# team-ergo-unipi/ergo_uvo

Hardware: AMD Instinct MI355X
Metric: stereo frame-pairs/sec (detect+match+pose) @1920x1080, 3k kpts (higher is better)
Workload: dtype f32+f64

## Files before the change

ergo_uvo_amd/csrc/ctx.hip:

```cpp
#include "uvo_ctx.h"
#include "uvo_pix.h"
#include <pthread.h>
#include "uvo_epnp.h"
#include <string.h>
#include <sched.h>
#include <atomic>
#include <math.h>
#include <float.h>
#include <new>
#include <algorithm>
namespace uvo { extern bool g_bdbg; extern std::atomic<double> g_bstat[16]; double now_us(); void operator+=(std::atomic<double>& a, double v); }

using namespace uvo;

struct uvo_ctx : public uvo::Ctx {};

namespace {
uvo_status abi_caught(uvo_ctx* c) noexcept
{
    uvo_status st = UVO_HIP_ERROR;
    const char* what = "unexpected C++ exception inside libuvo_hip";
    static thread_local char text[160];
    try { throw; }
    catch (const std::bad_alloc&) { st = UVO_CAPACITY; what = "out of host memory (std::bad_alloc) inside libuvo_hip"; }
// ... 116 lines not shown
static int stereo_a_streams(const uvo::Ctx* m, int depth) { return a_per_lane(m, depth) ? depth : a_shared_streams(m); }
static int stereo_a_slot(const uvo::Ctx* m, int depth, int lane, long long launch) { return a_per_lane(m, depth) ? lane : (int)(launch % a_shared_streams(m)); }
static void assign_entry_streams(uvo::Ctx* m, uvo::Ctx* L, bool stereo)
{
    if (L->assigned_seq == m->sh->plan_seq) return;
    L->assigned_seq = m->sh->plan_seq;
    const int depth = (int)m->sh->lanes.size();
    if (!stereo) { L->stream = slot_stream(m, 0, L->lane_id); L->pnp_stream = slot_stream(m, 1, L->lane_id); return; }
    L->stream = slot_stream(m, 0, stereo_a_slot(m, depth, L->lane_id, m->sh->a_launch++));
    L->pnp_stream = slot_stream(m, 1, m->sh->shared_slots ? (int)(m->sh->plan_seq % m->sh->n_b) : L->lane_id);
}
static void assign_idle_streams(uvo::Ctx* m)
{
    const int depth = (int)m->sh->lanes.size();
    m->sh->shared_slots = shared_layout(depth);
    m->sh->n_b = std::min((int)Shared::kMaxDepth, m->sh->max_b + 1);
    if (const char* e = getenv("UVO_B_STREAMS")) m->sh->n_b = std::min((int)Shared::kMaxDepth, std::max(1, atoi(e)));
    m->sh->a_launch = 0;
    if (m->sh->shared_slots) for (int i = 0; i < m->sh->n_b; i++) (void)slot_stream(m, 1, i);
    for (uvo::Ctx* l : m->sh->lanes) {
        l->stream = slot_stream(m, 0, stereo_a_slot(m, depth, l->lane_id, l->lane_id));
        l->pnp_stream = slot_stream(m, 1, m->sh->shared_slots ? l->lane_id % m->sh->n_b : l->lane_id);
        l->assigned_seq = -1;
    }
}

static const char* unsupported_params(const uvo_params* p)
{
    if (p->ITERATIONS_COUNT > 0 && p->PNP_METHOD_FLAG != 1)
        return "PNP_METHOD_FLAG: uvo_params takes only 1 (cv::SOLVEPNP_EPNP, the value shipped in stereo_VO_parameters.yaml); 2 (P3P), 3 (DLS) and 4 (UPNP) "
               "are set with uvo_ctx_set_pnp_method, 0 (ITERATIVE), 5 (AP3P) and above are not implemented";
    if (p->USE_EXTRINSIC_GUESS != 0) return "USE_EXTRINSIC_GUESS: only false is implemented (EPnP ignores the guess)";
    return nullptr;
}

static thread_local const char* t_create_refusal = nullptr;

static uvo_status create_one(const uvo_params* p, int device, int max_w, int max_h, int max_kpts, uvo_ctx** out, int lane = 0, Shared* sh = nullptr)
{
    if (!out) return UVO_INVALID_ARG;
    *out = nullptr;
    t_create_refusal = p ? unsupported_params(p) : nullptr;
    if (!p || max_w < 16 || max_h < 16 || max_kpts < 16 || t_create_refusal) return UVO_INVALID_ARG;
    int ndev = 0;
    if (hipGetDeviceCount(&ndev) != hipSuccess || ndev <= 0 || device < 0 || device >= ndev) return UVO_NO_DEVICE;
    if (hipSetDevice(device) != hipSuccess) return UVO_HIP_ERROR;
    uvo_ctx* c = new (std::nothrow) uvo_ctx();
    if (!c) return UVO_HIP_ERROR;
    c->sh = sh ? sh : new (std::nothrow) Shared();
    if (!c->sh) { delete c; return UVO_HIP_ERROR; }
    c->p = *p; c->device = device; c->max_w = max_w; c->max_h = max_h; c->cap = max_kpts; c->lane_id = lane;
    const size_t cap = (size_t)max_kpts;
    const size_t npx = (size_t)max_w * max_h, nsum = (size_t)(max_w + 1) * (max_h + 1);
    const int nstrip = (max_h + 7) / 8;
    c->colpart_stride = ((max_w + 1 + 2047) / 2048) * 2048;
    const size_t nchunks = (cap + 127) / 128;
    hipError_t e = hipSuccess;
#define A(expr) do { if (e == hipSuccess) e = (expr); } while (0)
    if (lane != 0) { c->stream = c->sh->slot_streams[0][0]; c->pnp_stream = c->sh->slot_streams[1][0]; }
    else { A(stream_acquire(device, 0, 0, &c->sh->slot_streams[0][0])); c->stream = c->sh->slot_streams[0][0]; }
    A(hipEventCreate(&c->ev0)); A(hipEventCreate(&c->ev1));
    c->plane_pw = ((max_w + 1 + 3) / 4 + 1 + 1) & ~1;
    c->plane_stride = c->plane_pw * ((max_h + 1 + 3) / 4 + 1);
    for (int i = 0; i < 2; i++) {
        A(dalloc(&c->d_planes[i], (size_t)16 * c->plane_stride));
        if (e == hipSuccess) e = hipMemset(c->d_planes[i], 0, sizeof(int32_t) * 16 * c->plane_stride);
        A(dalloc(&c->d_img[i], npx)); A(dalloc(&c->d_sum_base[i], nsum + 2 * kSumPad));
        if (e == hipSuccess) { e = hipMemset(c->d_sum_base[i], 0, sizeof(int32_t) * (nsum + 2 * kSumPad)); c->d_sum[i] = c->d_sum_base[i] + kSumPad; }
        A(dalloc(&c->d_cand[i], cap)); A(dalloc(&c->det[i].kps, cap)); A(dalloc(&c->det[i].desc, cap * 128));
        A(dalloc(&c->d_tmp_desc[i], cap * 128)); A(dalloc(&c->d_matches[i], cap));
        A(dalloc(&c->d_as_kpsL[i], cap)); A(dalloc(&c->d_as_kpsR[i], cap)); A(dalloc(&c->d_as_descL[i], cap * 128));
        A(dalloc(&c->d_as_pts4[i], cap)); A(dalloc(&c->d_as_cam1[i], cap * 3)); A(dalloc(&c->d_as_flag[i], cap));
    }
    c->surv_cap = 4 * (int)cap; A(dalloc(&c->d_surv, (size_t)c->surv_cap));
    A(dalloc(&c->d_colpart, (size_t)2 * nstrip * c->colpart_stride));
    A(dalloc(&c->d_DW, 400)); A(dalloc(&c->d_rank, cap * 2)); A(dalloc(&c->d_big_par, cap * 4)); A(dalloc(&c->d_big_patch, cap * 2 * 448));
    A(dalloc(&c->d_mpart, 2 * nchunks * cap)); A(dalloc(&c->d_mscratch, 2 * (nchunks + 4))); A(dalloc(&c->d_knn_idx, 2 * cap * 2)); A(dalloc(&c->d_knn_dist, 2 * cap * 2));
    A(dalloc(&c->d_x1, cap)); A(dalloc(&c->d_x2, cap)); A(dalloc(&c->d_xc, cap)); A(dalloc(&c->d_pts4, cap));
    A(dalloc(&c->d_cam1, cap * 3)); A(dalloc(&c->d_flag, cap)); A(dalloc(&c->d_tmp_idx, cap)); A(dalloc(&c->d_tmp_row, cap));
    if (const char* ww = getenv("UVO_WORKER_WAIT")) c->worker_wait = !strcmp(ww, "spin") ? 0 : (!strcmp(ww, "block-all") ? 2 : ((!strcmp(ww, "sleep") || !strcmp(ww, "block")) ? 3 : 1));
    c->wait_eff.store(c->worker_wait == 0 ? 0 : (c->worker_wait == 2 ? 2 : 1), std::memory_order_relaxed);
    A(hipEventCreateWithFlags(&c->evBlock, hipEventDisableTiming | hipEventBlockingSync));
    A(hipEventCreateWithFlags(&c->evPoll, hipEventDisableTiming));
    A(hipEventCreateWithFlags(&c->evB, hipEventDisableTiming | (c->worker_wait == 2 ? hipEventBlockingSync : 0)));
    for (int i = 0; i < 2; i++) {
        A(dalloc(&c->d_good_pts[i], cap * 3)); A(dalloc(&c->d_good_idx[i], cap));
        A(dalloc(&c->d_opts[i], cap * 3)); A(dalloc(&c->d_ipts[i], cap));
        A(hipEventCreateWithFlags(&c->evA[i], hipEventDisableTiming | ((i == 0 && c->worker_wait == 2) ? hipEventBlockingSync : 0)));
        A(hipHostMalloc(reinterpret_cast<void**>(&c->h_countsA[i]), sizeof(int) * CN_TOTAL));
    }
    A(hipEventCreateWithFlags(&c->evAS, hipEventDisableTiming));
    A(hipEventCreateWithFlags(&c->evSync, hipEventDisableTiming));
    A(hipEventCreateWithFlags(&c->evProducer, hipEventDisableTiming));
    A(hipEventCreateWithFlags(&c->evDet, hipEventDisableTiming)); A(hipEventCreateWithFlags(&c->evPrevRead, hipEventDisableTiming));
    if (lane == 0) { A(stream_acquire(device, 1, 0, &c->sh->slot_streams[1][0])); c->pnp_stream = c->sh->slot_streams[1][0]; }
    A(dalloc(&c->d_countsB, (size_t)4)); A(hipHostMalloc(reinterpret_cast<void**>(&c->h_countsB), sizeof(int) * 4));
    A(dalloc(&c->d_counts, (size_t)CN_TOTAL));
    A(dalloc(&c->d_subsets, (size_t)kMaxHyp * 5)); A(dalloc(&c->d_models, (size_t)kMaxHyp * 6)); A(dalloc(&c->d_hcount, (size_t)kMaxHyp));
    A(dalloc(&c->d_inliers, cap)); A(dalloc(&c->d_refit, cap * 21)); A(dalloc(&c->d_pose, (size_t)6));
    A(hipHostMalloc(reinterpret_cast<void**>(&c->h_counts), sizeof(int) * CN_TOTAL));
    A(hipHostMalloc(reinterpret_cast<void**>(&c->h_subsets), sizeof(int) * kMaxHyp * 5));
    A(hipHostMalloc(reinterpret_cast<void**>(&c->h_hcount), sizeof(int) * kMaxHyp));
    A(hipHostMalloc(reinterpret_cast<void**>(&c->h_pose), sizeof(double) * 6));
    A(dalloc(&c->d_rng_raw, (size_t)1024)); A(hipMalloc(&c->d_spec, 64)); A(hipHostMalloc(&c->h_spec, 64));
#undef A
    if (e != hipSuccess) { destroy_one(c); return UVO_HIP_ERROR; }
    c->d_cand_n = c->d_counts + CN_CAND0;
    c->det[0].n = c->d_counts + CN_NL; c->det[1].n = c->d_counts + CN_NR;
    c->d_nmatch = c->d_counts + CN_M;
    c->d_as_n = c->d_counts + CN_AS0;
    c->d_big_n = c->d_counts + CN_BIG0;
    if (surf_build_area_tables(c) != UVO_OK) { destroy_one(c); return UVO_HIP_ERROR; }
    {
        std::vector<unsigned> raw(1024);
        uint64_t state = (uint64_t)-1;
        for (auto& v : raw) v = rng_next(state);
        if (hipMemcpy(c->d_rng_raw, raw.data(), sizeof(unsigned) * raw.size(), hipMemcpyHostToDevice) != hipSuccess ||
            hipMemset(c->d_spec, 0, 64) != hipSuccess) { destroy_one(c); return UVO_HIP_ERROR; }
        memset(c->h_spec, 0, 64);
    }
    make_desc_weights(c->h_DW);
    if (hipMemcpy(c->d_DW, c->h_DW, sizeof(float) * 400, hipMemcpyHostToDevice) != hipSuccess ||
        hipMemset(c->d_rank, 0, sizeof(int) * cap * 2) != hipSuccess ||
        hipMemset(c->d_counts, 0, sizeof(int) * CN_TOTAL) != hipSuccess) { destroy_one(c); return UVO_HIP_ERROR; }
    if (getenv("UVO_TRACE") && trace_alloc(c) != hipSuccess) { destroy_one(c); return UVO_HIP_ERROR; }
    try { c->err.reserve(256); c->worker = std::thread(lane_worker, c); }
    catch (...) { destroy_one(c); return UVO_HIP_ERROR; }
    *out = c;
// ... 123 lines not shown
    if (st != UVO_OK) { uvo_ctx* made = *out; *out = nullptr; destroy_ctx(made); }
    return st;
} UVO_ABI_CATCH(nullptr)

extern "C" uvo_status uvo_stereo_set_depth(uvo_ctx* c, int depth)
try {
    if (!c) return UVO_INVALID_ARG;
    (void)hipSetDevice(c->device);
    return set_depth(c, depth);
} UVO_ABI_CATCH(c)

static void destroy_ctx(uvo_ctx* c)
{
    if (uvo::g_bdbg && uvo::g_bstat[4].load() > 0) {
        const double n = uvo::g_bstat[4].load();
        fprintf(stderr, "[uvo] stage B over %.0f calls, host wall us per call: wait-for-A %.1f | hyp+score to sync %.1f | host scan + refit launch %.1f | refit to sync %.1f | semaphore wait %.1f\n",
                n, uvo::g_bstat[0].load() / n, uvo::g_bstat[1].load() / n, uvo::g_bstat[2].load() / n, uvo::g_bstat[3].load() / n, uvo::g_bstat[5].load() / n);
        fprintf(stderr, "[uvo] uvo_stereo_submit host wall: %.1f us per pair over %.0f pairs\n", uvo::g_bstat[6].load() / std::max(1.0, uvo::g_bstat[7].load()), uvo::g_bstat[7].load());
        const double np = std::max(1.0, uvo::g_bstat[7].load());
        fprintf(stderr, "[uvo]   of which: upload %.1f | a_overlap wait %.1f | detector launches %.1f | matcher .. extract_3Dpoints launches %.1f\n",
                uvo::g_bstat[8].load() / np, uvo::g_bstat[9].load() / np, uvo::g_bstat[10].load() / np, uvo::g_bstat[11].load() / np);
    }
    write_trace(c);
    for (size_t i = c->sh->lanes.size(); i > 1; i--) destroy_one(static_cast<uvo_ctx*>(c->sh->lanes[i - 1]));
    c->sh->lanes.clear();
    destroy_one(c);
}
extern "C" void uvo_ctx_destroy(uvo_ctx* c)
try { if (c) destroy_ctx(c); } UVO_ABI_CATCH_VOID(c)

static void destroy_one(uvo_ctx* c)
{
    if (!c) return;
    (void)hipSetDevice(c->device);
    if (c->worker.joinable()) {
        { std::lock_guard<std::mutex> lk(c->mu); c->quit = true; }
        c->cv.notify_all();
        c->worker.join();
    }
    sync_owned_streams(c);
    for (int i = 0; i < 2; i++) {
        (void)hipFree(c->d_img[i]); (void)hipFree(c->d_sum_base[i]); (void)hipFree(c->d_planes[i]); (void)hipFree(c->d_cand[i]); (void)hipFree(c->det[i].kps);
        (void)hipFree(c->det[i].desc); (void)hipFree(c->d_tmp_desc[i]); (void)hipFree(c->d_matches[i]);
        (void)hipFree(c->d_as_kpsL[i]); (void)hipFree(c->d_as_kpsR[i]); (void)hipFree(c->d_as_descL[i]);
        (void)hipFree(c->d_as_pts4[i]); (void)hipFree(c->d_as_cam1[i]); (void)hipFree(c->d_as_flag[i]);
    }
    mono_ws_free(c);
    pre_ws_free(c);
    frames_ws_free(c);
    codec_ws_free(c);
    sift_ws_free(c);
    akaze_ws_free(c);
    orb_ws_free(c);
    void* ptrs[] = { c->d_hess_order, c->d_gen_tab, c->d_gen_planes, c->d_surv, c->d_octpat, c->d_colpart, c->d_DW, c->d_rank, c->d_big_par, c->d_big_patch, c->d_area_tabs, c->d_area_iscale, c->d_ori_w, c->d_mpart, c->d_mscratch, c->d_knn_idx, c->d_knn_dist, c->d_x1, c->d_x2, c->d_xc, c->d_pts4, c->d_cam1,
                     c->d_flag, c->d_tmp_idx, c->d_tmp_row, c->d_good_pts[0], c->d_good_pts[1], c->d_good_idx[0], c->d_good_idx[1], c->d_opts[0], c->d_opts[1],
                     c->d_ipts[0], c->d_ipts[1], c->d_counts, c->d_countsB, c->d_subsets, c->d_models,
                     c->d_hcount, c->d_inliers, c->d_refit, c->d_pose };
    for (void* p : ptrs) (void)hipFree(p);
    (void)hipHostFree(c->h_counts); (void)hipHostFree(c->h_subsets); (void)hipHostFree(c->h_hcount); (void)hipHostFree(c->h_pose);
    (void)hipHostFree(c->h_countsB); (void)hipHostFree(c->h_spec); (void)hipFree(c->d_rng_raw); (void)hipFree(c->d_spec);
    for (int i = 0; i < 2; i++) { (void)hipHostFree(c->h_countsA[i]); if (c->evA[i]) (void)hipEventDestroy(c->evA[i]); }
    if (c->evAS) (void)hipEventDestroy(c->evAS);
    if (c->evBlock) (void)hipEventDestroy(c->evBlock);
    if (c->evPoll) (void)hipEventDestroy(c->evPoll);
    if (c->evB) (void)hipEventDestroy(c->evB);
    if (c->evSync) (void)hipEventDestroy(c->evSync);
    if (c->evProducer) (void)hipEventDestroy(c->evProducer);
    for (auto& r : c->trace) for (int k = 0; k < 8; k++) if (r.ev[k]) (void)hipEventDestroy(r.ev[k]);
    if (c->evDet) (void)hipEventDestroy(c->evDet);
    if (c->evPrevRead) (void)hipEventDestroy(c->evPrevRead);
    if (c->ev0) (void)hipEventDestroy(c->ev0);
    if (c->ev1) (void)hipEventDestroy(c->ev1);
    if (c->lane_id == 0) {
        for (int role = 0; role < 2; role++) for (int i = 0; i < Shared::kMaxDepth; i++) { stream_release(c->device, role, i, c->sh->slot_streams[role][i]); c->sh->slot_streams[role][i] = nullptr; }
        delete c->sh;
    }
    delete c;
}

extern "C" const char* uvo_last_error(const uvo_ctx* c) { return c ? c->err.c_str() : (t_create_refusal ? t_create_refusal : "null context"); }
extern "C" void* uvo_ctx_stream(uvo_ctx* c) { return c ? (void*)c->stream : nullptr; }
extern "C" uvo_status uvo_ctx_set_params(uvo_ctx* c, const uvo_params* p)
try {
    if (!c || !p) return UVO_INVALID_ARG;
    if (c->sh->n_pending != 0) { c->err = "parameters cannot change while pairs are in flight"; return UVO_INVALID_ARG; }
    if (const char* why = unsupported_params(p)) { c->err = why; return UVO_INVALID_ARG; }
    if ((p->SURF_EXTENDED != 0) != (c->p.SURF_EXTENDED != 0) && (c->sh->vo_initialized || c->sh->mono_initialized)) {
        c->err = "SURF_EXTENDED changes the descriptor width: the previous frame's descriptors held by the running VO loop would not match (uvo_stereo_reset / uvo_mono_reset first)";
        return UVO_INVALID_ARG;
    }
    for (Ctx* l : c->sh->lanes) l->p = *p;
    return UVO_OK;
} UVO_ABI_CATCH(c)
extern "C" uvo_status uvo_ctx_set_producer_stream(uvo_ctx* c, void* hip_stream, int enabled)
try {
    if (!c) return UVO_INVALID_ARG;
    c->sh->producer_stream = static_cast<hipStream_t>(hip_stream); c->sh->has_producer = enabled != 0;
    return UVO_OK;
} UVO_ABI_CATCH(c)
extern "C" uvo_status uvo_device_alloc(uvo_ctx* c, size_t bytes, void** out)
try {
    if (!c) return UVO_INVALID_ARG;
    if (!out || bytes == 0) { c->err = "uvo_device_alloc: NULL result pointer or zero bytes"; return UVO_INVALID_ARG; }
    *out = nullptr;
    (void)hipSetDevice(c->device);
    UVO_HIP_TRY(c, hipMalloc(out, bytes));
    return UVO_OK;
// ... 2047 lines not shown
```

ergo_uvo_amd/csrc/surf.hip:

```cpp
#include "uvo_ctx.h"
#include <type_traits>
#include <string.h>
#include "uvo_math.h"
#include <algorithm>
#include <utility>
#include <vector>
#include <string>

namespace uvo {

struct ImgPair { const uint8_t* img[2]; int32_t* sum[2]; int32_t* planes[2]; int pw, pstride; int* cand_n; int* big_n; int* surv_n; };
struct AreaTab;
struct CandOut { uvo_keypoint* cand[2]; int* count; int cap; };
struct SurvOut { Survivor* list; int* count; int cap; };
static_assert(sizeof(Survivor) == 128, "a survivor record is 32 words");
struct SortArgs { const uvo_keypoint* cand[2]; const int* cand_n; uvo_keypoint* out[2]; int* out_n[2]; int* rank; int cap;
                  int4* big_par; int* big_n; int* gate_nqa; int gate_min_features; };
struct DescArgs { const uint8_t* img[2]; uvo_keypoint* kps[2]; float* desc[2]; const int* n[2]; const float* DW;
                  const int4* big_par; const int* big_n; const int* big_large; int cap;
                  const AreaTab* tabs; const int* iscale;
                  int extended;
                  const int32_t* sum[2]; const float* ori_w; int* ori_drop; };
struct LaneArgs { ImgPair ip; int32_t* part; SurvOut sv; CandOut out; SortArgs sa; DescArgs da; uint8_t* patch; const int4* big_in; int4* big_out; int* big_large; };
static const int kStripRows = 8;
static const int kStripCols = 2048;

__device__ __forceinline__ void strip_row_prefix(const uint8_t* img, int w, int h, int y0, int c0, int (*wt)[4], int (&carry)[kStripRows],
                                                 unsigned (&lo)[kStripRows], unsigned (&hi)[kStripRows], int (&E)[kStripRows])
{
    const int tid = threadIdx.x, lane = tid & 63, wv = tid >> 6;
    const bool vec8 = (w & 7) == 0;
#pragma unroll
    for (int r = 0; r < kStripRows; r++) {
        const int y = y0 + r;
        lo[r] = hi[r] = 0;
        if (y < h && c0 < w) {
            const uint8_t* src = img + (size_t)y * w + c0;
            if (vec8) { const uint2 v = *reinterpret_cast<const uint2*>(src); lo[r] = v.x; hi[r] = v.y; }
            else {
                for (int k = 0; k < 8; k++) if (c0 + k < w) { if (k < 4) lo[r] |= (unsigned)src[k] << (8 * k); else hi[r] |= (unsigned)src[k] << (8 * (k - 4)); }
            }
        }
    }
    int local[kStripRows], inc[kStripRows];
#pragma unroll
    for (int r = 0; r < kStripRows; r++) inc[r] = local[r] = (int)__builtin_amdgcn_sad_u8(lo[r], 0u, __builtin_amdgcn_sad_u8(hi[r], 0u, 0u));
#pragma unroll
    for (int r = 0; r < kStripRows; r++) {
        int v = inc[r];
        v += __builtin_amdgcn_update_dpp(0, v, 0x111, 0xf, 0xf, false);
        v += __builtin_amdgcn_update_dpp(0, v, 0x112, 0xf, 0xf, false);
        v += __builtin_amdgcn_update_dpp(0, v, 0x114, 0xf, 0xf, false);
        v += __builtin_amdgcn_update_dpp(0, v, 0x118, 0xf, 0xf, false);
        v += __builtin_amdgcn_update_dpp(0, v, 0x142, 0xa, 0xf, false);
        v += __builtin_amdgcn_update_dpp(0, v, 0x143, 0xc, 0xf, false);
        inc[r] = v;
    }
    if (lane == 63) {
#pragma unroll
        for (int r = 0; r < kStripRows; r++) wt[r][wv] = inc[r];
    }
    __syncthreads();
#pragma unroll
    for (int r = 0; r < kStripRows; r++) {
        const int t0 = wt[r][0], t1 = wt[r][1], t2 = wt[r][2], t3 = wt[r][3];
        const int base = carry[r] + (wv > 0 ? t0 : 0) + (wv > 1 ? t1 : 0) + (wv > 2 ? t2 : 0);
        E[r] = base + inc[r] - local[r];
        carry[r] += t0 + t1 + t2 + t3;
    }
}
__device__ __forceinline__ int packed_px(unsigned lo, unsigned hi, int k) { return (int)(((k < 4 ? lo : hi) >> (8 * (k & 3))) & 255u); }

__global__ __launch_bounds__(256) void k_integral_strip_sums(LaneArgs LA, int w, int h, int cstride, int nstrip)
{
    const ImgPair& ip = LA.ip; int32_t* part = LA.part;
    const int strip = blockIdx.x, im = blockIdx.y, tid = threadIdx.x;
    __shared__ int wt[kStripRows][4];
    int carry[kStripRows];
#pragma unroll
    for (int r = 0; r < kStripRows; r++) carry[r] = 0;
    int32_t* dst = part + ((size_t)im * nstrip + strip) * cstride;
    for (int cb = 0; cb <= w; cb += kStripCols) {
        unsigned lo[kStripRows], hi[kStripRows]; int E[kStripRows];
        strip_row_prefix(ip.img[im], w, h, strip * kStripRows, cb + 8 * tid, wt, carry, lo, hi, E);
        int cs[8] = {0, 0, 0, 0, 0, 0, 0, 0};
#pragma unroll
        for (int r = 0; r < kStripRows; r++) {
            int run = E[r];
#pragma unroll
            for (int k = 0; k < 8; k++) { cs[k] += run; run += packed_px(lo[r], hi[r], k); }
        }
        int4* d4 = reinterpret_cast<int4*>(dst + cb + 8 * tid);
        d4[0] = make_int4(cs[0], cs[1], cs[2], cs[3]); d4[1] = make_int4(cs[4], cs[5], cs[6], cs[7]);
        __syncthreads();
    }
    if (strip == 0 && tid == 0) { ip.cand_n[im] = 0; ip.big_n[im] = 0; if (im == 0) { *ip.surv_n = 0; ip.surv_n[CN_ORI_DROP - CN_SURV] = 0; } }
}

__global__ __launch_bounds__(256) void k_integral_strip_scan(LaneArgs LA, int cstride, int nstrip, int w)
{
    int32_t* part = LA.part;
    const int tid = threadIdx.x, xl = tid & 31, g = tid >> 5, x = blockIdx.x * 32 + xl, im = blockIdx.y;
    __shared__ int gsum[8][32];
    const int per = (nstrip + 7) / 8, s0 = g * per, s1 = min(nstrip, s0 + per);
    int32_t* p = part + (size_t)im * nstrip * cstride + x;
    const bool live = x <= w;
    int tot = 0;
#pragma unroll 8
    for (int sI = s0; sI < s1; sI++) tot += live ? p[(size_t)sI * cstride] : 0;
    gsum[g][xl] = tot;
    __syncthreads();
    int acc = 0;
    for (int k = 0; k < g; k++) acc += gsum[k][xl];
    if (!live) return;
#pragma unroll 8
    for (int sI = s0; sI < s1; sI++) { const int v = p[(size_t)sI * cstride]; p[(size_t)sI * cstride] = acc; acc += v; }
}

__global__ __launch_bounds__(256) void k_integral_strip_final(LaneArgs LA, int w, int h, int cstride, int nstrip)
{
    const ImgPair& ip = LA.ip; const int32_t* part = LA.part;
    const int strip = blockIdx.x, im = blockIdx.y, tid = threadIdx.x;
    const int sw = w + 1, y0 = strip * kStripRows;
    __shared__ int wt[kStripRows][4];
    __shared__ __align__(16) int rowbuf[kStripRows / 2][kStripCols];
    int carry[kStripRows];
#pragma unroll
    for (int r = 0; r < kStripRows; r++) carry[r] = 0;
    const int32_t* src = part + ((size_t)im * nstrip + strip) * cstride;
    int32_t* sum = ip.sum[im];
    int32_t* planes = ip.planes[im];
    for (int cb = 0; cb <= w; cb += kStripCols) {
        const int c0 = cb + 8 * tid;
        const int4* s4 = reinterpret_cast<const int4*>(src + c0);
        const int4 a0 = s4[0], a1 = s4[1];
        unsigned lo[kStripRows], hi[kStripRows]; int E[kStripRows];
        strip_row_prefix(ip.img[im], w, h, y0, c0, wt, carry, lo, hi, E);
        int acc[8] = { a0.x, a0.y, a0.z, a0.w, a1.x, a1.y, a1.z, a1.w };
#pragma unroll
        for (int half = 0; half < 2; half++) {
#pragma unroll
            for (int rr = 0; rr < kStripRows / 2; rr++) {
                const int r = half * (kStripRows / 2) + rr, ys = y0 + r + 1;
                int run = E[r];
#pragma unroll
                for (int k = 0; k < 8; k++) { acc[k] += run; run += packed_px(lo[r], hi[r], k); }
                int4* rb = reinterpret_cast<int4*>(&rowbuf[rr][8 * tid]);
                rb[0] = make_int4(acc[0], acc[1], acc[2], acc[3]); rb[1] = make_int4(acc[4], acc[5], acc[6], acc[7]);
                if (((r + 1) & 3) != 2 && ys <= h && c0 <= w) {
                    int32_t* pl = planes + (size_t)((ys & 3) * 4) * ip.pstride + (size_t)(ys >> 2) * ip.pw + (c0 >> 2);
                    if (c0 + 7 <= w) {
#pragma unroll
                        for (int rx = 0; rx < 4; rx++) if (rx != 2) *reinterpret_cast<int2*>(pl + (size_t)rx * ip.pstride) = make_int2(acc[rx], acc[rx + 4]);
                    } else {
#pragma unroll
                        for (int k = 0; k < 8; k++) if ((k & 3) != 2 && c0 + k <= w) pl[(size_t)(k & 3) * ip.pstride + (k >> 2)] = acc[k];
                    }
                }
            }
            __syncthreads();
#pragma unroll
            for (int rr = 0; rr < kStripRows / 2; rr++) {
                const int ys = y0 + half * (kStripRows / 2) + rr + 1;
                if (ys <= h) {
                    int32_t* drow = sum + (size_t)ys * sw + cb;
#pragma unroll
                    for (int j = 0; j < 8; j++) { const int xs = tid + 256 * j; if (cb + xs <= w) drow[xs] = rowbuf[rr][xs]; }
                }
            }
            __syncthreads();
        }
    }
    if (strip == 0) for (int x = tid; x < sw; x += 256) sum[x] = 0;
}

struct LayerPat {
    int dx1[10], dy1[10], dx2[10], dy2[10];
    float w[10];
    int size, margin, samples_i, samples_j;
};
struct OctavePat {
    LayerPat L[5];
    int step, rows, cols;
    int lo, hi;
    int nms_margin[3];
    int octave;
};

struct OctDims { struct { int samples_i, samples_j; } L[5]; int rows, cols, nms_margin[3], octave; };
struct HessDims { OctDims o[4]; };
static void make_pattern(int size, LayerPat* lp)
{
    static const int dx_s[3][5]  = { {0, 2, 3, 7, 1}, {3, 2, 6, 7, -2}, {6, 2, 9, 7, 1} };
    static const int dy_s[3][5]  = { {2, 0, 7, 3, 1}, {2, 3, 7, 6, -2}, {2, 6, 7, 9, 1} };
    static const int dxy_s[4][5] = { {1, 1, 4, 4, 1}, {5, 1, 8, 4, -1}, {1, 5, 4, 8, -1}, {5, 5, 8, 8, 1} };
    float ratio = (float)size / 9;
    for (int k = 0; k < 10; k++) {
        const int* s = k < 3 ? dx_s[k] : k < 6 ? dy_s[k - 3] : dxy_s[k - 6];
        int dx1 = cv_round_f(ratio * s[0]), dy1 = cv_round_f(ratio * s[1]);
        int dx2 = cv_round_f(ratio * s[2]), dy2 = cv_round_f(ratio * s[3]);
        lp->dx1[k] = dx1; lp->dy1[k] = dy1; lp->dx2[k] = dx2; lp->dy2[k] = dy2;
        lp->w[k] = s[4] / ((float)(dx2 - dx1) * (dy2 - dy1));
    }
    lp->size = size;
}

static void make_octave(int octave, int nOctaveLayers, int w, int h, OctavePat* op)
{
    int step = 1 << octave;
    op->step = step; op->rows = h / step; op->cols = w / step; op->octave = octave;
    op->lo = 0; op->hi = 0;
    for (int l = 0; l < 5; l++) {
        int size = (9 + 6 * l) << octave;
        LayerPat* lp = &op->L[l];
        make_pattern(size, lp);
        lp->margin = (size / 2) / step;
        bool fits = l < nOctaveLayers + 2 && size <= h && size <= w;
        lp->samples_i = fits ? 1 + (h - size) / step : 0;
        lp->samples_j = fits ? 1 + (w - size) / step : 0;
        int lo = -lp->margin * step, hi = lo + size;
// ... 1734 lines not shown
    }
    UVO_HIP_TRY(c, hipMalloc(reinterpret_cast<void**>(&c->d_area_tabs), tabs.size() * sizeof(AreaTab)));
    UVO_HIP_TRY(c, hipMalloc(reinterpret_cast<void**>(&c->d_area_iscale), isc.size() * sizeof(int)));
    UVO_HIP_TRY(c, hipMemcpy(c->d_area_tabs, tabs.data(), tabs.size() * sizeof(AreaTab), hipMemcpyHostToDevice));
    UVO_HIP_TRY(c, hipMemcpy(c->d_area_iscale, isc.data(), isc.size() * sizeof(int), hipMemcpyHostToDevice));
    {
        const int N = 2 * kOriRadius + 1;
        double t[N], sum = 0; float G[N], W[N * N];
        const double sigma = 2.5f, scale2X = -0.5 / (sigma * sigma);
        for (int i = 0; i < N; i++) { const double x = i - (N - 1) * 0.5; t[i] = exp(scale2X * x * x); sum += t[i]; }
        sum = 1. / sum;
        for (int i = 0; i < N; i++) G[i] = (float)(t[i] * sum);
        for (int i = 0; i < N; i++) for (int j = 0; j < N; j++) W[i * N + j] = G[i] * G[j];
        UVO_HIP_TRY(c, hipMalloc(reinterpret_cast<void**>(&c->d_ori_w), sizeof(W)));
        UVO_HIP_TRY(c, hipMemcpy(c->d_ori_w, W, sizeof(W), hipMemcpyHostToDevice));
    }
    return UVO_OK;
}

uvo_status surf_upload(Ctx* c, int slot, const uint8_t* gray, int w, int h, int stride, int mem)
{
    if (!gray || w <= 0 || h <= 0 || w > c->max_w || h > c->max_h || stride < w || slot < 0 || slot > 1) {
        c->err = "surf_upload: bad image geometry (w/h exceed the context's max_w/max_h?)";
        return UVO_INVALID_ARG;
    }
    if (slot == 1 && (w != c->img_w || h != c->img_h)) { c->err = "left/right image sizes differ"; return UVO_INVALID_ARG; }
    c->img_w = w; c->img_h = h;
    if (mem == UVO_MEM_DEVICE && stride == w && (reinterpret_cast<uintptr_t>(gray) & 15u) == 0) { c->img[slot] = gray; return UVO_OK; }
    UVO_HIP_TRY(c, hipMemcpy2DAsync(c->d_img[slot], w, gray, stride, w, h,
                                    mem == UVO_MEM_DEVICE ? hipMemcpyDeviceToDevice : hipMemcpyHostToDevice, c->stream));
    c->img[slot] = c->d_img[slot];
    return UVO_OK;
}

static LaneArgs lane_args(Ctx* c, int nimg, int gate_min_features)
{
    LaneArgs a;
    a.ip = ImgPair{ { c->img[0], c->img[1] }, { c->d_sum[0], c->d_sum[1] }, { c->d_planes[0], c->d_planes[1] }, c->plane_pw, c->plane_stride, c->d_cand_n, c->d_big_n, c->d_counts + CN_SURV };
    a.part = c->d_colpart;
    a.sv = SurvOut{ c->d_surv, c->d_counts + CN_SURV, c->surv_cap };
    a.out = CandOut{ { c->d_cand[0], c->d_cand[1] }, c->d_cand_n, c->cap };
    a.sa = SortArgs{ { c->d_cand[0], c->d_cand[1] }, c->d_cand_n, { c->det[0].kps, c->det[1].kps }, { c->det[0].n, c->det[1].n }, c->d_rank, c->cap, c->d_big_par, c->d_big_n,
                     gate_min_features >= 0 && nimg == 2 ? c->d_counts + CN_NQA : nullptr, gate_min_features };
    a.da = DescArgs{ { c->img[0], c->img[1] }, { c->det[0].kps, c->det[1].kps }, { c->det[0].desc, c->det[1].desc }, { c->det[0].n, c->det[1].n }, c->d_DW,
                     c->d_big_par + (size_t)2 * c->cap, c->d_big_n, c->d_counts + CN_BIGL0, c->cap,
                     c->d_area_tabs, c->d_area_iscale, c->p.SURF_EXTENDED ? 1 : 0, { c->d_sum[0], c->d_sum[1] }, c->d_ori_w, c->d_counts + CN_ORI_DROP };
    a.patch = c->d_big_patch;
    a.big_in = c->d_big_par; a.big_out = c->d_big_par + (size_t)2 * c->cap; a.big_large = c->d_counts + CN_BIGL0;
    return a;
}

static uvo_status surf_integral_launch(Ctx* c, const LaneArgs& LA, int nimg)
{
    const int w = c->img_w, h = c->img_h, sw = w + 1;
    const int nstrip = (h + kStripRows - 1) / kStripRows, cstride = c->colpart_stride;
    StageTimer t(c, ST_INTEGRAL);
    hipLaunchKernelGGL(k_integral_strip_sums, dim3(nstrip, nimg), dim3(256), 0, c->stream, LA, w, h, cstride, nstrip);
    hipLaunchKernelGGL(k_integral_strip_scan, dim3((sw + 31) / 32, nimg), dim3(256), 0, c->stream, LA, cstride, nstrip, w);
    hipLaunchKernelGGL(k_integral_strip_final, dim3(nstrip, nimg), dim3(256), 0, c->stream, LA, w, h, cstride, nstrip);
    UVO_HIP_TRY(c, hipGetLastError());
    return UVO_OK;
}
uvo_status surf_integral(Ctx* c, int nimg) { return surf_integral_launch(c, lane_args(c, nimg, -1), nimg); }

template <class K>
static hipError_t raise_dynamic_lds(const Ctx* c, K kern, size_t bytes, bool (&done)[64])
{
    bool& set = done[c->device & 63];
    if (set) return hipSuccess;
    const hipError_t e = hipFuncSetAttribute(reinterpret_cast<const void*>(kern), hipFuncAttributeMaxDynamicSharedMemorySize, (int)bytes);
    set = e == hipSuccess;
    return e;
}

struct MergedGrid { int nbx0, nb0, nbx1, nb1, nb23, total; P23Grid g; };
static const int kMergedTW0 = 64, kMergedTH0 = 32, kMergedTW1 = 32;
static MergedGrid merged_grid(const OctavePat* ops)
{
    constexpr int TW0 = kMergedTW0, TH0 = kMergedTH0, TW1 = kMergedTW1, TH1 = kO1TileRows;
    MergedGrid m;
    m.nbx0 = (ops[0].cols + TW0 - 3) / (TW0 - 2); m.nb0 = m.nbx0 * ((ops[0].rows + TH0 - 3) / (TH0 - 2));
    m.nbx1 = (ops[1].cols + TW1 - 3) / (TW1 - 2); m.nb1 = m.nbx1 * ((ops[1].rows + TH1 - 3) / (TH1 - 2));
    m.g.nbx2 = (ops[2].cols + 32 - 3) / (32 - 2); m.g.nb2 = m.g.nbx2 * ((ops[2].rows + 16 - 3) / (16 - 2));
    m.g.nbx3 = (ops[3].cols + 16 - 3) / (16 - 2); m.g.nb3 = m.g.nbx3 * ((ops[3].rows + 16 - 3) / (16 - 2));
    m.nb23 = m.g.nb2 + m.g.nb3; m.total = m.nb0 + m.nb1 + m.nb23;
    return m;
}

static bool general_path(const Ctx* c)
{
    return c->sh->surf_detection_path == 1 || c->p.SURF_OCTAVES_LAYERS != 3 || c->p.SURF_OCTAVES_NUMBER > 4;
}
static int widest_window(const Ctx* c, int w, int h)
{
    int win = 0;
    for (int o = 0; o < c->p.SURF_OCTAVES_NUMBER; o++)
        for (int l = 1; l <= c->p.SURF_OCTAVES_LAYERS; l++) {
            const int size = (9 + 6 * (l + 1)) << o;
            if (size > w || size > h) break;
            const float sc = (float)size * 1.2f / 9.0f;
            win = std::max(win, (int)((20 + 1) * sc));
        }
    return win;
}
static uvo_status general_prepare(Ctx* c, int w, int h)
{
    const int no = c->p.SURF_OCTAVES_NUMBER, nl = c->p.SURF_OCTAVES_LAYERS + 2;
    std::vector<unsigned char> raw(sizeof(GenTab), 0);
    GenTab* tab = reinterpret_cast<GenTab*>(raw.data());
    long long off = 0, need = 0;
    for (int o = 0; o < no; o++) for (int l = 0; l < nl; l++) {
        GenLayer* g = &tab->L[o * nl + l];
// ... 211 lines not shown
```

ergo_uvo_amd/csrc/uvo_ctx.h:

```cpp
#pragma once
#include <hip/hip_runtime.h>
#include <string>
#include <thread>
#include <mutex>
#include <condition_variable>
#include <atomic>
#include <vector>
#include <deque>
#include <stdint.h>
#include "../../include/uvo_hip.h"

namespace uvo {

#define UVO_HIP_TRY(c, expr)                                                                  \
    do {                                                                                      \
        hipError_t _e = (expr);                                                               \
        if (_e != hipSuccess) {                                                               \
            (c)->err = std::string(#expr) + ": " + hipGetErrorString(_e);                     \
            return UVO_HIP_ERROR;                                                             \
        }                                                                                     \
    } while (0)

#define UVO_TRY(expr)                                                                         \
    do { uvo_status _s = (expr); if (_s != UVO_OK) return _s; } while (0)

enum Stage {
    ST_INTEGRAL = 0, ST_HESSIAN_O0, ST_HESSIAN_O1, ST_HESSIAN_O2, ST_HESSIAN_O3, ST_SORT, ST_DESCRIPTOR, ST_MATCH, ST_MATCH_MERGE, ST_GATHER,
    ST_TRIANGULATE, ST_EXTRACT3D, ST_PNP_HYP, ST_PNP_SCORE, ST_PNP_REFIT, ST_COUNT
};
static const char* const kStageNames[ST_COUNT] = {
    "integral", "hessian_nms_o0", "hessian_nms_o1", "hessian_nms_o2", "hessian_nms_o3", "kp_sort", "descriptor64", "match_top2", "match_merge", "gather",
    "triangulate", "extract3d", "pnp_epnp5", "pnp_score", "pnp_refit"
};

enum { CN_T = 0, CN_G = 1, CN_NINL = 2, CN_NQA = 3, CN_NQB = 4, CN_MEFF = 5, CN_NL = 6, CN_NR = 7,
       CN_CAND0 = 8, CN_CAND1 = 9, CN_M = 10, CN_TRAW = 11, CN_AS0 = 12, CN_AS1 = 13, CN_BIG0 = 14, CN_BIG1 = 15, CN_SURV = 16, CN_BIGL0 = 17, CN_BIGL1 = 18, CN_ORI_DROP = 19, CN_TOTAL = 20 };
struct GateArgs { int mode; int* cn; int min_features, cap; int* as_curr_n; const int* as_prev_n; };

static const int kSumPad = 256;
static const int kMaxHyp = 2048;
static const int kBinRowWords = 16;

struct Survivor { int im, octave, L, i, j; float n9[27]; };

struct DetectSet {
    uvo_keypoint* kps;
    float* desc;
    int* n;
};

struct Ctx;
struct Shared {
    static const int kMaxDepth = 16;
    static const int kInflightMonoInit = -1, kInflightStereoInit = -2;
    std::vector<Ctx*> lanes;
    int next_lane = 0;
    int prev_lane = 0, prev_buf = 0;
    bool prev_sync = true;
    int inflight[kMaxDepth]; int n_pending = 0;
    long long n_submitted = 0, n_collected = 0;
    int last_lane = 0;
    long long plan_seq = 0;
    long long a_launch = 0;
    bool in_sync_step = false;
    int kp_hint = 0;
    bool vo_initialized = false;
    std::vector<uvo_dmatch> init_matches;
    bool rig_set = false;
    double t_prev_curr[3] = {0, 0, 0}, rvec[3] = {0, 0, 0}, tvec[3] = {0, 0, 0};
    std::deque<uvo_stereo_result> stereo_init_results;
    bool mono_cam_set = false, mono_initialized = false, mono_pipelined = false;
    int mono_use_essential = 1;
    double mono_R[9] = {1,0,0,0,1,0,0,0,1}, mono_t[3] = {0,0,0}, mono_SF = 1.0;
    std::deque<uvo_mono_result> mono_init_results;
    hipStream_t producer_stream = nullptr; bool has_producer = false;
    std::string warning, policy_text;
    double K_left[9], K_right[9], R_right[9], t_right[3], P_eye_left[12], P_right[12];
    double mono_K[9];
    int stage_b_mode = -1;
    double cpu_budget = 0;
    int a_overlap = 2;
    int a_overlap_mono = 4;
    int max_b = 3;
    int max_b_mono = 10;
    int detector = 0;
    int pnp_method = 1;
    int mono_pose_stage = 0;
    int surf_detection_path = 0;
    bool shared_slots = false;
    int n_b = 1;
    hipStream_t slot_streams[2][kMaxDepth] = {};
    std::mutex b_mu; std::condition_variable b_cv;
    int b_running = 0;
    long long b_seq = 0;
};

struct Ctx {
    uvo_params p;
    int device = 0, max_w = 0, max_h = 0, cap = 0;
    hipStream_t stream = nullptr;
    std::string err;
    hipEvent_t evProducer = nullptr;

    uint8_t* d_img[2] = {nullptr, nullptr};
    const uint8_t* img[2] = {nullptr, nullptr};
    int32_t* d_sum[2] = {nullptr, nullptr};
    int32_t* d_sum_base[2] = {nullptr, nullptr};
    int32_t* d_colpart = nullptr;
    int colpart_stride = 0;
    int32_t* d_planes[2] = {nullptr, nullptr};
    int plane_pw = 0, plane_stride = 0;
    uvo_keypoint* d_cand[2] = {nullptr, nullptr};
    int* d_cand_n = nullptr;
    Survivor* d_surv = nullptr; int surv_cap = 0;
    void* d_octpat = nullptr;
    std::vector<unsigned char> h_octpat;
    uint32_t* d_hess_order = nullptr; size_t d_hess_order_cap = 0;
    std::vector<uint32_t> h_hess_order; int hess_order_key[3] = {0, 0, 0};
    void* d_gen_tab = nullptr; std::vector<unsigned char> h_gen_tab;
    float* d_gen_planes = nullptr; size_t gen_planes_cap = 0; long long gen_img_floats = 0;
    int4* d_big_par = nullptr; int* d_big_n = nullptr;
    struct AreaTab* d_area_tabs = nullptr;
    float* d_ori_w = nullptr;
    int* d_area_iscale = nullptr;
    uint8_t* d_big_patch = nullptr;
    int* d_rank = nullptr;
    DetectSet det[2];
    int img_w = 0, img_h = 0;
    float h_DW[400];
    float* d_DW = nullptr;

    float4* d_mpart = nullptr;
    float* d_mscratch = nullptr;
    int* d_knn_idx = nullptr;  float* d_knn_dist = nullptr;
    float* d_tmp_desc[2] = {nullptr, nullptr};
    uvo_dmatch* d_matches[2] = {nullptr, nullptr};
    int* d_nmatch = nullptr;

    uvo_keypoint* d_as_kpsL[2] = {nullptr, nullptr};
    uvo_keypoint* d_as_kpsR[2] = {nullptr, nullptr};
    float* d_as_descL[2] = {nullptr, nullptr};
    int* d_as_n = nullptr;
    float4* d_as_pts4[2] = {nullptr, nullptr};  double* d_as_cam1[2] = {nullptr, nullptr};  int* d_as_flag[2] = {nullptr, nullptr};

    uvo_point2f *d_x1 = nullptr, *d_x2 = nullptr, *d_xc = nullptr;
    float4* d_pts4 = nullptr;
    double* d_cam1 = nullptr;
    int* d_flag = nullptr;
    double* d_good_pts[2] = {nullptr, nullptr};  int* d_good_idx[2] = {nullptr, nullptr};
    float* d_opts[2] = {nullptr, nullptr};  uvo_point2f* d_ipts[2] = {nullptr, nullptr};
    int* d_tmp_idx = nullptr;
    int* d_tmp_row = nullptr;
    int* d_counts = nullptr;
    int* h_counts = nullptr;

    int* d_subsets = nullptr;
    int* h_subsets = nullptr;
    double* d_models = nullptr;
    int* d_hcount = nullptr;  int* h_hcount = nullptr;
    int* d_inliers = nullptr;
    double* d_refit = nullptr;
// ... 221 lines not shown
```

Measured before the change: 3984.

## Restructure SURF integral image into two-pass grouped column-sum scheme with 16-bit partials

Replaces the three-kernel integral image pipeline (strip sums, strip scan, final) with two kernels. The first computes per-strip column sums inside groups of 16 strips in LDS and stores 16-bit intra-group prefixes plus group totals. The final kernel then reconstructs the column carry by summing the preceding group totals. It also narrows the partial buffers to uint16, which halves that traffic, and vectorizes the integral row stores with alignment handling. The carry reconstruction is redundant: each strip re-reads all earlier group totals, so the work grows with image height, and there is added edge-handling complexity.

```diff
diff --git a/ergo_uvo_amd/csrc/ctx.hip b/ergo_uvo_amd/csrc/ctx.hip
--- a/ergo_uvo_amd/csrc/ctx.hip
+++ b/ergo_uvo_amd/csrc/ctx.hip
@@ -192,7 +192,7 @@
     c->p = *p; c->device = device; c->max_w = max_w; c->max_h = max_h; c->cap = max_kpts; c->lane_id = lane;
     const size_t cap = (size_t)max_kpts;
     const size_t npx = (size_t)max_w * max_h, nsum = (size_t)(max_w + 1) * (max_h + 1);
-    const int nstrip = (max_h + 7) / 8;
+    const int nstrip = (max_h + kStripRows - 1) / kStripRows, ngroup = (nstrip + kStripGroup - 1) / kStripGroup;
     c->colpart_stride = ((max_w + 1 + 2047) / 2048) * 2048;
     const size_t nchunks = (cap + 127) / 128;
     hipError_t e = hipSuccess;
@@ -214,6 +214,7 @@
     }
     c->surv_cap = 4 * (int)cap; A(dalloc(&c->d_surv, (size_t)c->surv_cap));
     A(dalloc(&c->d_colpart, (size_t)2 * nstrip * c->colpart_stride));
+    A(dalloc(&c->d_coltot, (size_t)2 * ngroup * c->colpart_stride));
     A(dalloc(&c->d_DW, 400)); A(dalloc(&c->d_rank, cap * 2)); A(dalloc(&c->d_big_par, cap * 4)); A(dalloc(&c->d_big_patch, cap * 2 * 448));
     A(dalloc(&c->d_mpart, 2 * nchunks * cap)); A(dalloc(&c->d_mscratch, 2 * (nchunks + 4))); A(dalloc(&c->d_knn_idx, 2 * cap * 2)); A(dalloc(&c->d_knn_dist, 2 * cap * 2));
     A(dalloc(&c->d_x1, cap)); A(dalloc(&c->d_x2, cap)); A(dalloc(&c->d_xc, cap)); A(dalloc(&c->d_pts4, cap));
@@ -443,7 +444,7 @@
     sift_ws_free(c);
     akaze_ws_free(c);
     orb_ws_free(c);
-    void* ptrs[] = { c->d_hess_order, c->d_gen_tab, c->d_gen_planes, c->d_surv, c->d_octpat, c->d_colpart, c->d_DW, c->d_rank, c->d_big_par, c->d_big_patch, c->d_area_tabs, c->d_area_iscale, c->d_ori_w, c->d_mpart, c->d_mscratch, c->d_knn_idx, c->d_knn_dist, c->d_x1, c->d_x2, c->d_xc, c->d_pts4, c->d_cam1,
+    void* ptrs[] = { c->d_hess_order, c->d_gen_tab, c->d_gen_planes, c->d_surv, c->d_octpat, c->d_colpart, c->d_coltot, c->d_DW, c->d_rank, c->d_big_par, c->d_big_patch, c->d_area_tabs, c->d_area_iscale, c->d_ori_w, c->d_mpart, c->d_mscratch, c->d_knn_idx, c->d_knn_dist, c->d_x1, c->d_x2, c->d_xc, c->d_pts4, c->d_cam1,
                      c->d_flag, c->d_tmp_idx, c->d_tmp_row, c->d_good_pts[0], c->d_good_pts[1], c->d_good_idx[0], c->d_good_idx[1], c->d_opts[0], c->d_opts[1],
                      c->d_ipts[0], c->d_ipts[1], c->d_counts, c->d_countsB, c->d_subsets, c->d_models,
                      c->d_hcount, c->d_inliers, c->d_refit, c->d_pose };
diff --git a/ergo_uvo_amd/csrc/surf.hip b/ergo_uvo_amd/csrc/surf.hip
--- a/ergo_uvo_amd/csrc/surf.hip
+++ b/ergo_uvo_amd/csrc/surf.hip
@@ -21,14 +21,25 @@
                   const AreaTab* tabs; const int* iscale;
                   int extended;
                   const int32_t* sum[2]; const float* ori_w; int* ori_drop; };
-struct LaneArgs { ImgPair ip; int32_t* part; SurvOut sv; CandOut out; SortArgs sa; DescArgs da; uint8_t* patch; const int4* big_in; int4* big_out; int* big_large; };
-static const int kStripRows = 8;
+struct LaneArgs { ImgPair ip; uint16_t* part; SurvOut sv; CandOut out; SortArgs sa; DescArgs da; uint8_t* patch; const int4* big_in; int4* big_out; int* big_large; };
 static const int kStripCols = 2048;
-
-__device__ __forceinline__ void strip_row_prefix(const uint8_t* img, int w, int h, int y0, int c0, int (*wt)[4], int (&carry)[kStripRows],
-                                                 unsigned (&lo)[kStripRows], unsigned (&hi)[kStripRows], int (&E)[kStripRows])
-{
-    const int tid = threadIdx.x, lane = tid & 63, wv = tid >> 6;
+static const int kStripBufRows = 2;
+static const int kGroupCols = 128;
+static_assert(kStripRows % 4 == 0 && kStripRows % kStripBufRows == 0, "plane rows go by (r + 1) & 3; whole LDS batches");
+static_assert(kStripGroup * (kGroupCols / 8) == 256 && kStripGroup * kStripRows * 255 < 65536, "a thread per strip and column octet; a group's column sums fit 16 bits");
+
+__device__ __forceinline__ int wave_inclusive_scan(int v)
+{
+    v += __builtin_amdgcn_update_dpp(0, v, 0x111, 0xf, 0xf, false);
+    v += __builtin_amdgcn_update_dpp(0, v, 0x112, 0xf, 0xf, false);
+    v += __builtin_amdgcn_update_dpp(0, v, 0x114, 0xf, 0xf, false);
+    v += __builtin_amdgcn_update_dpp(0, v, 0x118, 0xf, 0xf, false);
+    v += __builtin_amdgcn_update_dpp(0, v, 0x142, 0xa, 0xf, false);
+    v += __builtin_amdgcn_update_dpp(0, v, 0x143, 0xc, 0xf, false);
+    return v;
+}
+__device__ __forceinline__ void strip_load(const uint8_t* img, int w, int h, int y0, int c0, unsigned (&lo)[kStripRows], unsigned (&hi)[kStripRows])
+{
     const bool vec8 = (w & 7) == 0;
 #pragma unroll
     for (int r = 0; r < kStripRows; r++) {
@@ -42,20 +53,15 @@
             }
         }
     }
+}
+__device__ __forceinline__ void strip_row_prefix(int (*wt)[4], int (&carry)[kStripRows], const unsigned (&lo)[kStripRows], const unsigned (&hi)[kStripRows], int (&E)[kStripRows])
+{
+    const int tid = threadIdx.x, lane = tid & 63, wv = tid >> 6;
     int local[kStripRows], inc[kStripRows];
 #pragma unroll
-    for (int r = 0; r < kStripRows; r++) inc[r] = local[r] = (int)__builtin_amdgcn_sad_u8(lo[r], 0u, __builtin_amdgcn_sad_u8(hi[r], 0u, 0u));
-#pragma unroll
-    for (int r = 0; r < kStripRows; r++) {
-        int v = inc[r];
-        v += __builtin_amdgcn_update_dpp(0, v, 0x111, 0xf, 0xf, false);
-        v += __builtin_amdgcn_update_dpp(0, v, 0x112, 0xf, 0xf, false);
-        v += __builtin_amdgcn_update_dpp(0, v, 0x114, 0xf, 0xf, false);
-        v += __builtin_amdgcn_update_dpp(0, v, 0x118, 0xf, 0xf, false);
-        v += __builtin_amdgcn_update_dpp(0, v, 0x142, 0xa, 0xf, false);
-        v += __builtin_amdgcn_update_dpp(0, v, 0x143, 0xc, 0xf, false);
-        inc[r] = v;
-    }
+    for (int r = 0; r < kStripRows; r++) local[r] = (int)__builtin_amdgcn_sad_u8(lo[r], 0u, __builtin_amdgcn_sad_u8(hi[r], 0u, 0u));
+#pragma unroll
+    for (int r = 0; r < kStripRows; r++) inc[r] = wave_inclusive_scan(local[r]);
     if (lane == 63) {
 #pragma unroll
         for (int r = 0; r < kStripRows; r++) wt[r][wv] = inc[r];
@@ -71,77 +77,84 @@
 }
 __device__ __forceinline__ int packed_px(unsigned lo, unsigned hi, int k) { return (int)(((k < 4 ? lo : hi) >> (8 * (k & 3))) & 255u); }
 
-__global__ __launch_bounds__(256) void k_integral_strip_sums(LaneArgs LA, int w, int h, int cstride, int nstrip)
-{
-    const ImgPair& ip = LA.ip; int32_t* part = LA.part;
-    const int strip = blockIdx.x, im = blockIdx.y, tid = threadIdx.x;
+__global__ __launch_bounds__(256) void k_integral_group_sums(LaneArgs LA, uint16_t* tot16, int w, int h, int cstride, int nstrip, int ngroup)
+{
+    const ImgPair& ip = LA.ip; uint16_t* part16 = LA.part;
+    const int tid = threadIdx.x, t = tid & (kGroupCols / 8 - 1), sl = tid / (kGroupCols / 8);
+    const int group = blockIdx.x, im = blockIdx.z, strip = group * kStripGroup + sl, c0 = blockIdx.y * kGroupCols + 8 * t;
+    __shared__ uint4 colsum[kStripGroup][kGroupCols / 8];
+    unsigned lo[kStripRows], hi[kStripRows];
+    strip_load(ip.img[im], w, h, strip * kStripRows, c0, lo, hi);
+    uint4 own = make_uint4(0u, 0u, 0u, 0u);
+#pragma unroll
+    for (int r = 0; r < kStripRows; r++) {
+        own.x += lo[r] & 0x00ff00ffu; own.y += (lo[r] >> 8) & 0x00ff00ffu;
+        own.z += hi[r] & 0x00ff00ffu; own.w += (hi[r] >> 8) & 0x00ff00ffu;
+    }
+    colsum[sl][t] = own;
+    __syncthreads();
+    uint4 a = make_uint4(0u, 0u, 0u, 0u);
+#pragma unroll
+    for (int k = 0; k < kStripGroup - 1; k++) if (k < sl) { const uint4 v = colsum[k][t]; a.x += v.x; a.y += v.y; a.z += v.z; a.w += v.w; }
+    if (c0 < w) {
+        if (strip < nstrip) *reinterpret_cast<uint4*>(part16 + ((size_t)im * nstrip + strip) * cstride + c0) = a;
+        if (sl == kStripGroup - 1) *reinterpret_cast<uint4*>(tot16 + ((size_t)im * ngroup + group) * cstride + c0) = make_uint4(a.x + own.x, a.y + own.y, a.z + own.z, a.w + own.w);
+    }
+    if (group == 0 && blockIdx.y == 0 && tid == 0) { ip.cand_n[im] = 0; ip.big_n[im] = 0; if (im == 0) { *ip.surv_n = 0; ip.surv_n[CN_ORI_DROP - CN_SURV] = 0; } }
+}
+
+__global__ __launch_bounds__(256) void k_integral_strip_final(LaneArgs LA, const uint16_t* tot16, int w, int h, int cstride, int nstrip, int ngroup)
+{
+    const ImgPair& ip = LA.ip;
+    const int strip = blockIdx.x, im = blockIdx.y, tid = threadIdx.x, wv = tid >> 6;
+    const int sw = w + 1, y0 = strip * kStripRows, group = strip / kStripGroup;
     __shared__ int wt[kStripRows][4];
-    int carry[kStripRows];
+    __shared__ int wtv[4];
+    __shared__ __align__(16) int rowbuf[kStripBufRows][kStripCols];
+    int carry[kStripRows], carryv = 0;
 #pragma unroll
     for (int r = 0; r < kStripRows; r++) carry[r] = 0;
-    int32_t* dst = part + ((size_t)im * nstrip + strip) * cstride;
-    for (int cb = 0; cb <= w; cb += kStripCols) {
-        unsigned lo[kStripRows], hi[kStripRows]; int E[kStripRows];
-        strip_row_prefix(ip.img[im], w, h, strip * kStripRows, cb + 8 * tid, wt, carry, lo, hi, E);
-        int cs[8] = {0, 0, 0, 0, 0, 0, 0, 0};
-#pragma unroll
-        for (int r = 0; r < kStripRows; r++) {
-            int run = E[r];
-#pragma unroll
-            for (int k = 0; k < 8; k++) { cs[k] += run; run += packed_px(lo[r], hi[r], k); }
-        }
-        int4* d4 = reinterpret_cast<int4*>(dst + cb + 8 * tid);
-        d4[0] = make_int4(cs[0], cs[1], cs[2], cs[3]); d4[1] = make_int4(cs[4], cs[5], cs[6], cs[7]);
-        __syncthreads();
-    }
-    if (strip == 0 && tid == 0) { ip.cand_n[im] = 0; ip.big_n[im] = 0; if (im == 0) { *ip.surv_n = 0; ip.surv_n[CN_ORI_DROP - CN_SURV] = 0; } }
-}
-
-__global__ __launch_bounds__(256) void k_integral_strip_scan(LaneArgs LA, int cstride, int nstrip, int w)
-{
-    int32_t* part = LA.part;
-    const int tid = threadIdx.x, xl = tid & 31, g = tid >> 5, x = blockIdx.x * 32 + xl, im = blockIdx.y;
-    __shared__ int gsum[8][32];
-    const int per = (nstrip + 7) / 8, s0 = g * per, s1 = min(nstrip, s0 + per);
-    int32_t* p = part + (size_t)im * nstrip * cstride + x;
-    const bool live = x <= w;
-    int tot = 0;
-#pragma unroll 8
-    for (int sI = s0; sI < s1; sI++) tot += live ? p[(size_t)sI * cstride] : 0;
-    gsum[g][xl] = tot;
-    __syncthreads();
-    int acc = 0;
-    for (int k = 0; k < g; k++) acc += gsum[k][xl];
-    if (!live) return;
-#pragma unroll 8
-    for (int sI = s0; sI < s1; sI++) { const int v = p[(size_t)sI * cstride]; p[(size_t)sI * cstride] = acc; acc += v; }
-}
-
-__global__ __launch_bounds__(256) void k_integral_strip_final(LaneArgs LA, int w, int h, int cstride, int nstrip)
-{
-    const ImgPair& ip = LA.ip; const int32_t* part = LA.part;
-    const int strip = blockIdx.x, im = blockIdx.y, tid = threadIdx.x;
-    const int sw = w + 1, y0 = strip * kStripRows;
-    __shared__ int wt[kStripRows][4];
-    __shared__ __align__(16) int rowbuf[kStripRows / 2][kStripCols];
-    int carry[kStripRows];
-#pragma unroll
-    for (int r = 0; r < kStripRows; r++) carry[r] = 0;
-    const int32_t* src = part + ((size_t)im * nstrip + strip) * cstride;
+    const uint16_t* src16 = LA.part + ((size_t)im * nstrip + strip) * cstride;
+    const uint16_t* gtot16 = tot16 + (size_t)im * ngroup * cstride;
     int32_t* sum = ip.sum[im];
     int32_t* planes = ip.planes[im];
     for (int cb = 0; cb <= w; cb += kStripCols) {
         const int c0 = cb + 8 * tid;
-        const int4* s4 = reinterpret_cast<const int4*>(src + c0);
-        const int4 a0 = s4[0], a1 = s4[1];
         unsigned lo[kStripRows], hi[kStripRows]; int E[kStripRows];
-        strip_row_prefix(ip.img[im], w, h, y0, c0, wt, carry, lo, hi, E);
-        int acc[8] = { a0.x, a0.y, a0.z, a0.w, a1.x, a1.y, a1.z, a1.w };
-#pragma unroll
-        for (int half = 0; half < 2; half++) {
-#pragma unroll
-            for (int rr = 0; rr < kStripRows / 2; rr++) {
-                const int r = half * (kStripRows / 2) + rr, ys = y0 + r + 1;
+        strip_load(ip.img[im], w, h, y0, c0, lo, hi);
+        int V[8] = {0, 0, 0, 0, 0, 0, 0, 0};
+        if (c0 < w) {
+            for (int g0 = -1; g0 < group; g0 += 8) {
+                uint4 q[8];
+#pragma unroll
+                for (int k = 0; k < 8; k++) {
+                    const int g = g0 + k;
+                    q[k] = g < group ? *reinterpret_cast<const uint4*>(g < 0 ? src16 + c0 : gtot16 + (size_t)g * cstride + c0) : make_uint4(0u, 0u, 0u, 0u);
+                }
+#pragma unroll
+                for (int k = 0; k < 8; k++) {
+                    V[0] += (int)(q[k].x & 0xffffu); V[2] += (int)(q[k].x >> 16); V[1] += (int)(q[k].y & 0xffffu); V[3] += (int)(q[k].y >> 16);
+                    V[4] += (int)(q[k].z & 0xffffu); V[6] += (int)(q[k].z >> 16); V[5] += (int)(q[k].w & 0xffffu); V[7] += (int)(q[k].w >> 16);
+                }
+            }
+        }
+        const int vloc = V[0] + V[1] + V[2] + V[3] + V[4] + V[5] + V[6] + V[7], vinc = wave_inclusive_scan(vloc);
+        if ((tid & 63) == 63) wtv[wv] = vinc;
+        strip_row_prefix(wt, carry, lo, hi, E);
+        int acc[8];
+        {
+            const int t0 = wtv[0], t1 = wtv[1], t2 = wtv[2], t3 = wtv[3];
+            acc[0] = carryv + (wv > 0 ? t0 : 0) + (wv > 1 ? t1 : 0) + (wv > 2 ? t2 : 0) + vinc - vloc;
+#pragma unroll
+            for (int k = 1; k < 8; k++) acc[k] = acc[k - 1] + V[k - 1];
+            carryv += t0 + t1 + t2 + t3;
+        }
+        const int ncol = min(kStripCols, sw - cb);
+#pragma unroll
+        for (int part_i = 0; part_i < kStripRows / kStripBufRows; part_i++) {
+#pragma unroll
+            for (int rr = 0; rr < kStripBufRows; rr++) {
+                const int r = part_i * kStripBufRows + rr, ys = y0 + r + 1;
                 int run = E[r];
 #pragma unroll
                 for (int k = 0; k < 8; k++) { acc[k] += run; run += packed_px(lo[r], hi[r], k); }
@@ -160,12 +173,20 @@
             }
             __syncthreads();
 #pragma unroll
-            for (int rr = 0; rr < kStripRows / 2; rr++) {
-                const int ys = y0 + half * (kStripRows / 2) + rr + 1;
+            for (int rr = 0; rr < kStripBufRows; rr++) {
+                const int ys = y0 + part_i * kStripBufRows + rr + 1;
                 if (ys <= h) {
                     int32_t* drow = sum + (size_t)ys * sw + cb;
-#pragma unroll
-                    for (int j = 0; j < 8; j++) { const int xs = tid + 256 * j; if (cb + xs <= w) drow[xs] = rowbuf[rr][xs]; }
+                    const int x0 = (4 - (int)((reinterpret_cast<uintptr_t>(drow) >> 2) & 3)) & 3;
+                    const int nq = ncol > x0 ? (ncol - x0) >> 2 : 0;
+#pragma unroll
+                    for (int j = 0; j < kStripCols / 4 / 256; j++) {
+                        const int q = tid + 256 * j, x = x0 + 4 * q;
+                        if (q < nq) *reinterpret_cast<int4*>(drow + x) = make_int4(rowbuf[rr][x], rowbuf[rr][x + 1], rowbuf[rr][x + 2], rowbuf[rr][x + 3]);
+                    }
+                    if (tid < x0 && tid < ncol) drow[tid] = rowbuf[rr][tid];
+                    const int xt = x0 + 4 * nq + tid - 64;
+                    if (tid >= 64 && tid < 67 && ncol > x0 && xt < ncol) drow[xt] = rowbuf[rr][xt];
                 }
             }
             __syncthreads();
@@ -2006,12 +2027,12 @@
 
 static uvo_status surf_integral_launch(Ctx* c, const LaneArgs& LA, int nimg)
 {
-    const int w = c->img_w, h = c->img_h, sw = w + 1;
+    const int w = c->img_w, h = c->img_h;
     const int nstrip = (h + kStripRows - 1) / kStripRows, cstride = c->colpart_stride;
     StageTimer t(c, ST_INTEGRAL);
-    hipLaunchKernelGGL(k_integral_strip_sums, dim3(nstrip, nimg), dim3(256), 0, c->stream, LA, w, h, cstride, nstrip);
-    hipLaunchKernelGGL(k_integral_strip_scan, dim3((sw + 31) / 32, nimg), dim3(256), 0, c->stream, LA, cstride, nstrip, w);
-    hipLaunchKernelGGL(k_integral_strip_final, dim3(nstrip, nimg), dim3(256), 0, c->stream, LA, w, h, cstride, nstrip);
+    const int ngroup = (nstrip + kStripGroup - 1) / kStripGroup;
+    hipLaunchKernelGGL(k_integral_group_sums, dim3(ngroup, (w + kGroupCols - 1) / kGroupCols, nimg), dim3(256), 0, c->stream, LA, c->d_coltot, w, h, cstride, nstrip, ngroup);
+    hipLaunchKernelGGL(k_integral_strip_final, dim3(nstrip, nimg), dim3(256), 0, c->stream, LA, c->d_coltot, w, h, cstride, nstrip, ngroup);
     UVO_HIP_TRY(c, hipGetLastError());
     return UVO_OK;
 }
diff --git a/ergo_uvo_amd/csrc/uvo_ctx.h b/ergo_uvo_amd/csrc/uvo_ctx.h
--- a/ergo_uvo_amd/csrc/uvo_ctx.h
+++ b/ergo_uvo_amd/csrc/uvo_ctx.h
@@ -38,6 +38,8 @@
 struct GateArgs { int mode; int* cn; int min_features, cap; int* as_curr_n; const int* as_prev_n; };
 
 static const int kSumPad = 256;
+static const int kStripRows = 8;
+static const int kStripGroup = 16;
 static const int kMaxHyp = 2048;
 static const int kBinRowWords = 16;
 
@@ -106,7 +108,8 @@
     const uint8_t* img[2] = {nullptr, nullptr};
     int32_t* d_sum[2] = {nullptr, nullptr};
     int32_t* d_sum_base[2] = {nullptr, nullptr};
-    int32_t* d_colpart = nullptr;
+    uint16_t* d_colpart = nullptr;
+    uint16_t* d_coltot = nullptr;
     int colpart_stride = 0;
     int32_t* d_planes[2] = {nullptr, nullptr};
     int plane_pw = 0, plane_stride = 0;
```

New measurement: 3743. 6.1% lower.
